# qitianwu/SGFormer

Measured on NVIDIA H100. Metric: nodes/sec fwd+bwd, higher is better.
Workload: dtype bf16

## Files before the change

sgformer_b200/csrc/common.cuh:

```cuda
#pragma once
#include <cuda.h>
#include <cuda_bf16.h>
#include <cuda_runtime.h>
#include <stdint.h>

#define SGF_OK 0
#define SGF_ERR_ARG (-1)
#define SGF_ERR_UNSUPPORTED (-2)
#define SGF_ERR_DRIVER (-3)

#define SGF_CUDA_TRY(expr)                        \
    do {                                          \
        cudaError_t _e = (expr);                  \
        if (_e != cudaSuccess) return (int)_e;    \
    } while (0)

#define SGF_LAUNCH_CHECK()                        \
    do {                                          \
        cudaError_t _e = cudaGetLastError();      \
        if (_e != cudaSuccess) return (int)_e;    \
    } while (0)

namespace sgf {

// ... 100 lines not shown
}
__device__ __forceinline__ void mbar_arrive(uint64_t* bar) {
    asm volatile("mbarrier.arrive.shared::cta.b64 _, [%0];" :: "r"(smem_u32(bar)) : "memory");
}
__device__ __forceinline__ bool mbar_try_wait(uint64_t* bar, uint32_t parity) {
    uint32_t ok;
    asm volatile(
        "{\n\t.reg .pred P;\n\t"
        "mbarrier.try_wait.parity.shared::cta.b64 P, [%1], %2;\n\t"
        "selp.b32 %0, 1, 0, P;\n\t}\n"
        : "=r"(ok) : "r"(smem_u32(bar)), "r"(parity) : "memory");
    return ok != 0;
}
__device__ __forceinline__ void mbar_wait(uint64_t* bar, uint32_t parity) {
    uint32_t spins = 0;
    while (!mbar_try_wait(bar, parity)) {
        if (++spins > (1u << 26)) __trap();
    }
}

__device__ __forceinline__ void tma_prefetch_desc(const void* tmap) {
    asm volatile("prefetch.tensormap [%0];" :: "l"(tmap) : "memory");
}
__device__ __forceinline__ void tma_load_2d(void* smem_dst, const void* tmap, uint64_t* bar, int32_t c0, int32_t c1) {
    asm volatile(
        "cp.async.bulk.tensor.2d.shared::cluster.global.mbarrier::complete_tx::bytes [%0], [%1, {%3, %4}], [%2];"
        :: "r"(smem_u32(smem_dst)), "l"(tmap), "r"(smem_u32(bar)), "r"(c0), "r"(c1) : "memory");
}

__device__ __forceinline__ void tma_store_2d(const void* tmap, const void* smem_src, int32_t c0, int32_t c1) {
    asm volatile("cp.async.bulk.tensor.2d.global.shared::cta.bulk_group [%0, {%2, %3}], [%1];"
                 :: "l"(tmap), "r"(smem_u32(smem_src)), "r"(c0), "r"(c1) : "memory");
}
__device__ __forceinline__ void cp_async16(void* smem_dst, const void* gsrc) {
    const uint32_t s = static_cast<uint32_t>(__cvta_generic_to_shared(smem_dst));
    asm volatile("cp.async.cg.shared.global [%0], [%1], 16;" ::"r"(s), "l"(gsrc) : "memory");
}
__device__ __forceinline__ void cp_async_commit() { asm volatile("cp.async.commit_group;" ::: "memory"); }
template <int N>
__device__ __forceinline__ void cp_async_wait() {
    asm volatile("cp.async.wait_group %0;" ::"n"(N) : "memory");
}

__device__ __forceinline__ void bulk_commit() { asm volatile("cp.async.bulk.commit_group;" ::: "memory"); }
template <int N> __device__ __forceinline__ void bulk_wait_read() {
    asm volatile("cp.async.bulk.wait_group.read %0;" :: "n"(N) : "memory");
}
template <int N> __device__ __forceinline__ void bulk_wait() {
    asm volatile("cp.async.bulk.wait_group %0;" :: "n"(N) : "memory");
}
__device__ __forceinline__ void named_bar_sync(int id, int nthreads) {
    asm volatile("bar.sync %0, %1;" :: "r"(id), "r"(nthreads) : "memory");
}

__device__ __forceinline__ void wgmma_fence() { asm volatile("wgmma.fence.sync.aligned;" ::: "memory"); }
__device__ __forceinline__ void wgmma_commit() { asm volatile("wgmma.commit_group.sync.aligned;" ::: "memory"); }
template <int N> __device__ __forceinline__ void wgmma_wait() {
    asm volatile("wgmma.wait_group.sync.aligned %0;" :: "n"(N) : "memory");
}
template <int N> __device__ __forceinline__ void fence_regs(float (&d)[N]) {
#pragma unroll
    for (int i = 0; i < N; ++i) asm volatile("" : "+f"(d[i]) :: "memory");
}

template <int TA, int TB>
__device__ __forceinline__ void wgmma_n64(float (&d)[32], uint64_t da, uint64_t db, uint32_t scale_d) {
// ... 56 lines not shown
```

sgformer_b200/csrc/gemm_tc.cu:

```cuda
#include "common.cuh"
#include "launch_count.h"
#include "../../include/sgformer_b200.h"

#include <cstdlib>
#include <cstring>
#include <mutex>

namespace sgf {

typedef CUresult (*PFN_encodeTiled)(CUtensorMap*, CUtensorMapDataType, cuuint32_t, void*, const cuuint64_t*, const cuuint64_t*,
                                    const cuuint32_t*, const cuuint32_t*, CUtensorMapInterleave, CUtensorMapSwizzle,
                                    CUtensorMapL2promotion, CUtensorMapFloatOOBfill);
static PFN_encodeTiled get_encode() {
    static PFN_encodeTiled fn = nullptr;
    static std::once_flag once;
    std::call_once(once, [] {
        void* p = nullptr;
        cudaDriverEntryPointQueryResult q;
        if (cudaGetDriverEntryPoint("cuTensorMapEncodeTiled", &p, cudaEnableDefault, &q) == cudaSuccess &&
            q == cudaDriverEntryPointSuccess)
            fn = (PFN_encodeTiled)p;
    });
    return fn;
}
// ... 1 lines not shown
static int make_tmap_2d(CUtensorMap* tm, const void* base, int dtype, int64_t rows, int64_t cols, int64_t ld, int box_rows) {
    PFN_encodeTiled enc = get_encode();
    if (!enc) return SGF_ERR_DRIVER;
    const int es = dtype == 1 ? 2 : 4;
    if ((reinterpret_cast<uintptr_t>(base) & 15) || (ld * es) % 16 != 0 || rows <= 0 || cols <= 0 || box_rows <= 0 || box_rows > 256)
        return SGF_ERR_ARG;
    cuuint64_t gdim[2] = {(cuuint64_t)cols, (cuuint64_t)rows};
    cuuint64_t gstr[1] = {(cuuint64_t)ld * es};
    cuuint32_t box[2] = {(cuuint32_t)(128 / es), (cuuint32_t)box_rows};
    cuuint32_t estr[2] = {1u, 1u};
    CUresult r = enc(tm, dtype == 1 ? CU_TENSOR_MAP_DATA_TYPE_BFLOAT16 : CU_TENSOR_MAP_DATA_TYPE_FLOAT32, 2,
                     const_cast<void*>(base), gdim, gstr, box, estr, CU_TENSOR_MAP_INTERLEAVE_NONE,
                     CU_TENSOR_MAP_SWIZZLE_128B, CU_TENSOR_MAP_L2_PROMOTION_L2_128B, CU_TENSOR_MAP_FLOAT_OOB_FILL_NONE);
    return r == CUDA_SUCCESS ? SGF_OK : SGF_ERR_DRIVER;
}
static int make_tmap_bf16(CUtensorMap* tm, const void* base, int64_t rows, int64_t cols, int64_t ld, int box_rows) {
    return make_tmap_2d(tm, base, 1, rows, cols, ld, box_rows);
}

namespace nt {
constexpr int BM = 128, BK = 64, STAGES = 3;
constexpr int MMA_WARPS = 8;
constexpr int THREADS = 32 * (MMA_WARPS + 4);
constexpr int A_BYTES = BM * BK * 2;
constexpr int B_BYTES_MAX = (256 + 16) * BK * 2;
constexpr int STAGE_BYTES = A_BYTES + B_BYTES_MAX;
constexpr int WSTG_BYTES = 16 * 128;
constexpr int BAR_BYTES = 512;
constexpr int STAT_COLS = 1024;
constexpr int STAT_BYTES = 2 * STAT_COLS * 4;
constexpr int SMEM_BYTES = STAGES * STAGE_BYTES + MMA_WARPS * 2 * WSTG_BYTES + BAR_BYTES + STAT_BYTES + 1024;
constexpr int RES_BYTES = (256 + 16) * 256 * 2;
constexpr int RES_MAX_KB = 16;
constexpr int RES_STAGES = 3;
constexpr int SMEM_BYTES_RES = RES_BYTES + RES_STAGES * A_BYTES + MMA_WARPS * WSTG_BYTES + BAR_BYTES + STAT_BYTES + 1024;
static_assert(SMEM_BYTES <= 232448 && SMEM_BYTES_RES <= 232448, "exceeds the 227 KB of dynamic shared memory per CTA");

struct Seg {
    int a_idx, a_koff, b_idx, b_koff, k_blocks;
};
struct Params {
    int64_t rows;
    int n_out, bn_main, bn_pad, has_tail, n_blocks;
    int64_t num_tiles;
    int b_res;
    int64_t chunk;
    int n_seg, total_kb;
    Seg seg[SGF_MAX_SEG];
    int epi;
    void* out; int64_t ldo; int out_dtype;
    const float* bias;
    const void* aux; int64_t ld_aux; int aux_dtype;
    const float* row_scale;
    float alpha, beta;
    const float* alpha_dev; const float* beta_dev;
    int relu, accumulate;
    float nf; const float* nf_dev; float* den_out;
    const float* r1_row; const float* r1_col;
    int tma_store;
    float* col_sum; float* col_sumsq;
};
struct Tmaps {
    CUtensorMap a[SGF_MAX_SRC];
    CUtensorMap b[SGF_MAX_SRC];
    CUtensorMap tail;
    CUtensorMap out;
};

__device__ __forceinline__ float load1(const void* base, int dtype, int64_t off) {
    return dtype == 1 ? __bfloat162float(static_cast<const __nv_bfloat16*>(base)[off]) : static_cast<const float*>(base)[off];
}
__device__ __forceinline__ void store1(void* base, int dtype, int64_t off, float v) {
    if (dtype == 1) static_cast<__nv_bfloat16*>(base)[off] = __float2bfloat16_rn(v);
    else static_cast<float*>(base)[off] = v;
}
struct TileIter {
    const Params& p;
    bool started = false;
// ... 45 lines not shown

enum : int { F_BIAS = 1, F_AUX = 2, F_RELU = 4, F_ROWSCALE = 8, F_ACCUM = 16, F_R1 = 32, F_ATTN = 64, F_GENERIC = 128 };

template <bool GEN>
__device__ __forceinline__ void load_piece(const void* src, int dtype, int64_t ld, const int64_t* rows, const bool* row_ok,
                                           int col0, int n_out, bool nc, float* d) {
#pragma unroll
    for (int c = 0; c < 4; ++c)
#pragma unroll
        for (int s = 0; s < 2; ++s) {
            const int col = col0 + 8 * c;
            const int64_t off = rows[s] * ld + col;
            float a0 = 0.f, a1 = 0.f;
            if (!GEN) {
                if (row_ok[s]) {
                    const uint32_t* q = reinterpret_cast<const uint32_t*>(static_cast<const __nv_bfloat16*>(src) + off);
                    unpack_bf16x2(nc ? __ldg(q) : *q, a0, a1);
                }
            } else {
                if (row_ok[s] && col < n_out) a0 = load1(src, dtype, off);
                if (row_ok[s] && col + 1 < n_out) a1 = load1(src, dtype, off + 1);
            }
            d[4 * c + 2 * s] = a0;
            d[4 * c + 2 * s + 1] = a1;
        }
}

template <int F>
__global__ void __launch_bounds__(THREADS, 1) gemm_nt_kernel(const __grid_constant__ Tmaps tm, const __grid_constant__ Params p) {
    extern __shared__ uint8_t smem_raw[];
    uint8_t* smem = reinterpret_cast<uint8_t*>((reinterpret_cast<uintptr_t>(smem_raw) + 1023) & ~static_cast<uintptr_t>(1023));
    const bool res = p.b_res != 0;
    uint8_t* bres = smem;
    uint8_t* ring = res ? smem + RES_BYTES : smem;
    const int ring_stages = res ? RES_STAGES : STAGES;
    const int ring_stride = res ? A_BYTES : STAGE_BYTES;
    const int stg_per_warp = res ? 1 : 2;
    uint8_t* staging = ring + ring_stages * ring_stride;
    uint64_t* full = reinterpret_cast<uint64_t*>(staging + MMA_WARPS * stg_per_warp * WSTG_BYTES);
    uint64_t* empty = full + STAGES;
    uint64_t* bres_full = empty + STAGES;
    uint64_t* bres_empty = bres_full + RES_MAX_KB;
    float* stat_sm = reinterpret_cast<float*>(reinterpret_cast<uint8_t*>(full) + BAR_BYTES);
    static_assert((2 * STAGES + 2 * RES_MAX_KB) * 8 <= BAR_BYTES, "barrier area");
    static_assert(RES_STAGES <= STAGES, "ring barriers");
    const bool want_stats = p.col_sum != nullptr || p.col_sumsq != nullptr;

    const int warp = threadIdx.x >> 5;
    const int lane = threadIdx.x & 31;
    const uint32_t b_tx = p.bn_pad * BK * 2 + (p.has_tail ? 16 * BK * 2 : 0);
    if (want_stats)
        for (int i = threadIdx.x; i < 2 * STAT_COLS; i += THREADS) stat_sm[i] = 0.f;

    if (threadIdx.x == 0) {
        for (int i = 0; i < p.n_seg; ++i) {
            tma_prefetch_desc(&tm.a[p.seg[i].a_idx]);
            tma_prefetch_desc(&tm.b[p.seg[i].b_idx]);
        }
        if (p.has_tail) tma_prefetch_desc(&tm.tail);
        if (p.tma_store) tma_prefetch_desc(&tm.out);
        for (int s = 0; s < STAGES; ++s) { mbar_init(&full[s], 1); mbar_init(&empty[s], MMA_WARPS); }
        for (int s = 0; s < RES_MAX_KB; ++s) { mbar_init(&bres_full[s], 1); mbar_init(&bres_empty[s], MMA_WARPS); }
        fence_barrier_init();
    }
    __syncthreads();

    if (warp >= MMA_WARPS) {
        producer_regs();
        if (warp == MMA_WARPS && lane == 0) {
            int stage = 0; uint32_t phase = 0;
            TileIter ti(p);
            while (ti.next()) {
                int kbg = 0;
                for (int s = 0; s < p.n_seg; ++s) {
                    const Seg sg = p.seg[s];
                    for (int kb = 0; kb < sg.k_blocks; ++kb, ++kbg) {
                        mbar_wait(&empty[stage], phase ^ 1);
                        uint8_t* sa = ring + stage * ring_stride;
                        if (!res) {
                            uint8_t* sb = sa + A_BYTES;
                            mbar_arrive_expect_tx(&full[stage], A_BYTES + b_tx);
                            tma_load_2d(sa, &tm.a[sg.a_idx], &full[stage], sg.a_koff + kb * BK, ti.m_blk * BM);
                            tma_load_2d(sb, &tm.b[sg.b_idx], &full[stage], sg.b_koff + kb * BK, ti.n_blk * p.bn_main);
                            if (p.has_tail) tma_load_2d(sb + p.bn_pad * BK * 2, &tm.tail, &full[stage], sg.b_koff + kb * BK, 0);
                        } else {
                            mbar_arrive_expect_tx(&full[stage], A_BYTES);
                            tma_load_2d(sa, &tm.a[sg.a_idx], &full[stage], sg.a_koff + kb * BK, ti.m_blk * BM);
                            if (ti.first) {
                                mbar_wait(&bres_empty[kbg], (uint32_t)(ti.group & 1) ^ 1);
                                uint8_t* sb = bres + (size_t)kbg * b_tx;
                                mbar_arrive_expect_tx(&bres_full[kbg], b_tx);
                                tma_load_2d(sb, &tm.b[sg.b_idx], &bres_full[kbg], sg.b_koff + kb * BK, ti.n_blk * p.bn_main);
                                if (p.has_tail) tma_load_2d(sb + p.bn_pad * BK * 2, &tm.tail, &bres_full[kbg], sg.b_koff + kb * BK, 0);
                            }
// ... 9 lines not shown

    constexpr bool GEN = (F & F_GENERIC) != 0;
    const bool f_bias = GEN ? p.bias != nullptr : (F & F_BIAS) != 0;
    const bool f_aux = GEN ? p.aux != nullptr : (F & F_AUX) != 0;
    const bool f_relu = GEN ? p.relu != 0 : (F & F_RELU) != 0;
    const bool f_rs = GEN ? p.row_scale != nullptr : (F & F_ROWSCALE) != 0;
    const bool f_acc = GEN ? p.accumulate != 0 : (F & F_ACCUM) != 0;
    const bool f_r1 = GEN ? p.r1_row != nullptr : (F & F_R1) != 0;
    const bool f_attn = GEN ? (p.epi == SGF_EPI_ATTN_APPLY || p.epi == SGF_EPI_ATTN_GRAM) : (F & F_ATTN) != 0;
    const bool f_tma = GEN ? p.tma_store != 0 : true;
    const bool f_stats = GEN ? want_stats : false;
    const int out_dtype = GEN ? p.out_dtype : 1;
    const int wg = warp >> 2;
    const int wq = warp & 3;
    const int rr = lane >> 2;
    const int cq = 2 * (lane & 3);
    float alpha = p.alpha, beta = p.beta;
    if (p.alpha_dev) alpha *= *p.alpha_dev;
    if (p.beta_dev) beta *= *p.beta_dev;
    const float nfv = (f_attn && p.nf_dev) ? *p.nf_dev : p.nf;
    const int GW = out_dtype == 1 ? 64 : 32;
    const int ppg = GW / 32;
    const int n_pieces = (p.bn_main + 31) / 32;
    const int nch = p.bn_pad / 64;
    uint8_t* wstg = staging + warp * stg_per_warp * WSTG_BYTES;
    const uint32_t a_off = wg * 64 * BK * 2;

    float acc[4][32];
    float acct[8];
    uint32_t gcount = 0;
    int stage = 0; uint32_t phase = 0;
    TileIter ti(p);
    while (ti.next()) {
        for (int kbg = 0; kbg < p.total_kb; ++kbg) {
            if (res && ti.first) mbar_wait(&bres_full[kbg], (uint32_t)(ti.group & 1));
            mbar_wait(&full[stage], phase);
            const uint32_t sa = smem_u32(ring + stage * ring_stride) + a_off;
            const uint32_t sb = res ? smem_u32(bres) + (uint32_t)kbg * b_tx : smem_u32(ring + stage * ring_stride) + A_BYTES;
            wgmma_fence();
#pragma unroll
            for (int k = 0; k < BK / 16; ++k) {
                const uint64_t da = make_smem_desc_sw128(sa + k * 32, 16, 1024);
                const uint32_t sc = (kbg > 0 || k > 0) ? 1u : 0u;
#pragma unroll
                for (int j = 0; j < 4; ++j)
                    if (j < nch) wgmma_n64<0, 0>(acc[j], da, make_smem_desc_sw128(sb + j * 8192 + k * 32, 16, 1024), sc);
                if (p.has_tail) wgmma_n16<0, 0>(acct, da, make_smem_desc_sw128(sb + p.bn_pad * BK * 2 + k * 32, 16, 1024), sc);
            }
            wgmma_commit();
            wgmma_wait<0>();
#pragma unroll
            for (int j = 0; j < 4; ++j) fence_regs(acc[j]);
            fence_regs(acct);
            __syncwarp();
            if (lane == 0) {
                mbar_arrive(&empty[stage]);
                if (res && ti.last) mbar_arrive(&bres_empty[kbg]);
            }
            if (++stage == ring_stages) { stage = 0; phase ^= 1; }
        }

        const int m_blk = ti.m_blk, n_blk = ti.n_blk;
        const int64_t row_w = (int64_t)m_blk * BM + wg * 64 + wq * 16;
        const int64_t rows[2] = {row_w + rr, row_w + rr + 8};
        const bool row_ok[2] = {rows[0] < p.rows, rows[1] < p.rows};
        const int col_base = n_blk * p.bn_main;
        float rs[2] = {1.f, 1.f}, r1r[2] = {0.f, 0.f}, inv_den[2] = {1.f, 1.f};
#pragma unroll
        for (int s = 0; s < 2; ++s) {
            if (f_rs && row_ok[s]) rs[s] = p.row_scale[rows[s]];
            if (f_r1 && row_ok[s]) r1r[s] = p.r1_row[rows[s]];
        }
        if (f_attn) {
#pragma unroll
            for (int s = 0; s < 2; ++s) {
                const float den = __shfl_sync(0xffffffffu, acct[2 * s], lane & ~3) + nfv;
                inv_den[s] = 1.f / den;
                if (row_ok[s] && p.den_out && n_blk == 0 && (lane & 3) == 0) p.den_out[rows[s]] = den;
            }
        }
#pragma unroll
        for (int pc = 0; pc < 8; ++pc) {
            if (pc >= n_pieces) break;
            const int g = pc / ppg, pp = pc % ppg;
            const uint32_t buf = stg_per_warp == 2 ? (gcount & 1) : 0;
            if (f_tma && pp == 0) {
                if (lane == 0) {
                    if (stg_per_warp == 2) bulk_wait_read<1>(); else bulk_wait_read<0>();
                }
                __syncwarp();
            }
            float v[16];
#pragma unroll
            for (int i = 0; i < 16; ++i) v[i] = acc[pc >> 1][(pc & 1) * 16 + i];
            const int col0 = col_base + pc * 32 + cq;
            float ax[16], old[16];
            if (f_aux) load_piece<GEN>(p.aux, p.aux_dtype, p.ld_aux, rows, row_ok, col0, p.n_out, true, ax);
            if (f_acc) load_piece<GEN>(p.out, out_dtype, p.ldo, rows, row_ok, col0, p.n_out, false, old);
#pragma unroll
// ... 56 lines not shown
                        float s1 = 0.f, s2 = 0.f;
                        for (int r = 0; r < 16 && r < valid_rows; ++r) {
                            float x;
                            if (out_dtype == 1) {
                                const int chunk = (cg >> 3) ^ (r & 7);
                                x = __bfloat162float(*reinterpret_cast<const __nv_bfloat16*>(tile + r * 128 + chunk * 16 + (cg & 7) * 2));
                            } else {
                                const int chunk = (cg >> 2) ^ (r & 7);
                                x = *reinterpret_cast<const float*>(tile + r * 128 + chunk * 16 + (cg & 3) * 4);
                            }
                            s1 += x;
                            s2 += x * x;
                        }
                        atomicAdd(&stat_sm[colg], s1);
                        atomicAdd(&stat_sm[STAT_COLS + colg], s2);
                    }
                }
                ++gcount;
            }
        }
    }
    if (f_tma && lane == 0) bulk_wait<0>();
    if (f_stats) {
        named_bar_sync(3, 32 * MMA_WARPS);
        for (int i = threadIdx.x; i < p.n_out; i += 32 * MMA_WARPS) {
            if (p.col_sum) atomicAdd(&p.col_sum[i], stat_sm[i]);
            if (p.col_sumsq) atomicAdd(&p.col_sumsq[i], stat_sm[STAT_COLS + i]);
        }
    }
}
}

constexpr int FLUSH_KB = 16;
template <int BATCH>
__device__ __forceinline__ void flush_acc(float (&acc)[4][32], float* ws, int mp, int mrow, int cq, int j0, int ncols, bool add) {
#pragma unroll
    for (int j = 0; j < 4; ++j) {
        if (j < j0) continue;
#pragma unroll
        for (int i0 = 0; i0 < 32; i0 += BATCH) {
            float old[BATCH];
#pragma unroll
            for (int q = 0; q < BATCH; ++q) {
                const int i = i0 + q, col = 64 * j + 8 * (i >> 2) + cq + (i & 1);
                old[q] = (add && col < ncols) ? ws[(int64_t)col * mp + mrow + 8 * ((i >> 1) & 1)] : 0.f;
            }
#pragma unroll
            for (int q = 0; q < BATCH; ++q) {
                const int i = i0 + q, col = 64 * j + 8 * (i >> 2) + cq + (i & 1);
                if (col < ncols) ws[(int64_t)col * mp + mrow + 8 * ((i >> 1) & 1)] = add ? old[q] + acc[j][i] : acc[j][i];
                acc[j][i] = 0.f;
            }
        }
    }
}

namespace tn {
constexpr int BKN = 64, STAGES = 4, MMA_WARPS = 8, THREADS = 32 * (MMA_WARPS + 4);
constexpr int CHUNK_BYTES = 64 * BKN * 2;
constexpr int A_BYTES = 2 * CHUNK_BYTES;
constexpr int B_BYTES = 4 * CHUNK_BYTES;
constexpr int STAGE_BYTES = A_BYTES + B_BYTES;
constexpr int BAR_BYTES = 256;
constexpr int SMEM_BYTES = STAGES * STAGE_BYTES + BAR_BYTES + 1024;

struct Params {
    int64_t rows;
    int m, n, mp, n_chunks, un;
    int64_t kb_total;
    float* ws;
    int n_pairs;
    int a_off[SGF_TN_MAX_PAIRS], b_off[SGF_TN_MAX_PAIRS];
};
struct Tmaps {
    CUtensorMap a, b;
};

__global__ void __launch_bounds__(THREADS, 1) gemm_tn_kernel(const __grid_constant__ Tmaps tm, const __grid_constant__ Params p) {
    extern __shared__ uint8_t smem_raw[];
    uint8_t* smem = reinterpret_cast<uint8_t*>((reinterpret_cast<uintptr_t>(smem_raw) + 1023) & ~static_cast<uintptr_t>(1023));
    uint64_t* full = reinterpret_cast<uint64_t*>(smem + STAGES * STAGE_BYTES);
    uint64_t* empty = full + STAGES;

    const int warp = threadIdx.x >> 5;
    const int lane = threadIdx.x & 31;
    const int64_t per = p.kb_total / gridDim.y, rem = p.kb_total % gridDim.y;
    const int64_t kb0 = blockIdx.y * per + (blockIdx.y < rem ? blockIdx.y : rem);
    const int64_t kb1 = kb0 + per + (blockIdx.y < rem ? 1 : 0);
    const int m0 = blockIdx.x * 128;
    const int a_chunks = (p.m - m0) >= 128 ? 2 : ((p.m - m0) + 63) / 64;

    if (threadIdx.x == 0) {
        tma_prefetch_desc(&tm.a);
        tma_prefetch_desc(&tm.b);
        for (int s = 0; s < STAGES; ++s) { mbar_init(&full[s], 1); mbar_init(&empty[s], MMA_WARPS); }
        fence_barrier_init();
    }
    __syncthreads();

    if (warp >= MMA_WARPS) {
        producer_regs();
        if (warp == MMA_WARPS && lane == 0) {
            const uint32_t stage_tx = (a_chunks + p.n_chunks) * CHUNK_BYTES;
            int stage = 0; uint32_t phase = 0;
            for (int64_t kb = kb0; kb < kb1; ++kb) {
                for (int pr = 0; pr < p.n_pairs; ++pr) {
                    mbar_wait(&empty[stage], phase ^ 1);
                    uint8_t* sa = smem + stage * STAGE_BYTES;
                    uint8_t* sb = sa + A_BYTES;
                    mbar_arrive_expect_tx(&full[stage], stage_tx);
                    for (int c = 0; c < a_chunks; ++c)
                        tma_load_2d(sa + c * CHUNK_BYTES, &tm.a, &full[stage], p.a_off[pr] + m0 + c * 64, (int32_t)(kb * BKN));
                    for (int c = 0; c < p.n_chunks; ++c)
                        tma_load_2d(sb + c * CHUNK_BYTES, &tm.b, &full[stage], p.b_off[pr] + c * 64, (int32_t)(kb * BKN));
                    if (++stage == STAGES) { stage = 0; phase ^= 1; }
                }
            }
        }
        return;
    }
    consumer_regs();

    const int wg = warp >> 2, wq = warp & 3;
    const bool active = wg < a_chunks;
    float acc[4][32];
#pragma unroll
    for (int j = 0; j < 4; ++j)
#pragma unroll
        for (int i = 0; i < 32; ++i) acc[j][i] = 0.f;
    float* ws = p.ws + (int64_t)blockIdx.y * p.un * p.mp;
    const int mrow = m0 + wg * 64 + wq * 16 + (lane >> 2);
    const int cq = 2 * (lane & 3);
    bool flushed = false;
    int stage = 0; uint32_t phase = 0;
    for (int64_t kb = kb0; kb < kb1; ++kb) {
        for (int pr = 0; pr < p.n_pairs; ++pr) {
            mbar_wait(&full[stage], phase);
            if (active) {
                const uint32_t sa = smem_u32(smem + stage * STAGE_BYTES) + wg * CHUNK_BYTES;
                const uint32_t sb = smem_u32(smem + stage * STAGE_BYTES) + A_BYTES;
                wgmma_fence();
#pragma unroll
                for (int k = 0; k < BKN / 16; ++k) {
                    const uint64_t da = make_smem_desc_sw128(sa + k * 2048, CHUNK_BYTES, 1024);
#pragma unroll
                    for (int j = 0; j < 4; ++j)
                        if (j < p.n_chunks) wgmma_n64<1, 1>(acc[j], da, make_smem_desc_sw128(sb + j * CHUNK_BYTES + k * 2048, CHUNK_BYTES, 1024), 1u);
                }
                wgmma_commit();
                wgmma_wait<0>();
#pragma unroll
                for (int j = 0; j < 4; ++j) fence_regs(acc[j]);
            }
            __syncwarp();
            if (lane == 0) mbar_arrive(&empty[stage]);
            if (++stage == STAGES) { stage = 0; phase ^= 1; }
        }
        if (active && (kb - kb0 + 1) % FLUSH_KB == 0 && kb + 1 < kb1) {
            flush_acc<16>(acc, ws, p.mp, mrow, cq, 0, p.un, flushed);
            flushed = true;
        }
    }
    flush_acc<16>(acc, ws, p.mp, mrow, cq, 0, p.un, flushed);
}

__global__ void tn_reduce_kernel(const float* __restrict__ ws, int nparts, int mp, int un, int m, int n, float alpha,
                                 const float* __restrict__ alpha_dev, float beta, float* __restrict__ out, int64_t ldo, int transpose_out) {
    const int64_t total = (int64_t)n * mp;
    const float a = alpha * (alpha_dev ? *alpha_dev : 1.f);
    for (int64_t t = (int64_t)blockIdx.x * blockDim.x + threadIdx.x; t < total; t += (int64_t)gridDim.x * blockDim.x) {
        const int j = (int)(t / mp), i = (int)(t % mp);
        if (i >= m) continue;
        float s = 0.f;
        for (int c = 0; c < nparts; ++c) s += ws[((int64_t)c * un + j) * mp + i];
        float* o = transpose_out ? &out[(int64_t)j * ldo + i] : &out[(int64_t)i * ldo + j];
        *o = a * s + (beta != 0.f ? beta * *o : 0.f);
    }
}
}
namespace gramk {
constexpr int BKN = 64, MMA_WARPS = 8, THREADS = 32 * (MMA_WARPS + 4);
constexpr int CHUNK_BYTES = 64 * BKN * 2;
constexpr int ONES_BYTES = CHUNK_BYTES;
constexpr int BAR_BYTES = 256;
constexpr int SMEM_BUDGET = 200 * 1024;
constexpr int MAX_STAGES = 8;

struct Params {
    int64_t rows, kb_total;
    int h, chunks, m_blocks, un, mp, n_planes, stages;
    int plane_off[3];
    int n_pairs, pa[6], pb[6];
    float* ws;
};

__global__ void __launch_bounds__(THREADS, 1) gram_kernel(const __grid_constant__ CUtensorMap tm, const __grid_constant__ Params p) {
    extern __shared__ uint8_t smem_raw[];
    uint8_t* smem = reinterpret_cast<uint8_t*>((reinterpret_cast<uintptr_t>(smem_raw) + 1023) & ~static_cast<uintptr_t>(1023));
    const int c0 = blockIdx.x;
    const int nld = p.chunks - c0;
    const int plane_bytes = nld * CHUNK_BYTES;
    const int stage_stride = p.n_planes * p.chunks * CHUNK_BYTES;
    uint8_t* ones = smem + p.stages * stage_stride;
    uint64_t* full = reinterpret_cast<uint64_t*>(ones + ONES_BYTES);
    uint64_t* empty = full + MAX_STAGES;
    static_assert(2 * MAX_STAGES * 8 <= BAR_BYTES, "barrier area");

    const int warp = threadIdx.x >> 5;
    const int lane = threadIdx.x & 31;
    const int64_t per = p.kb_total / gridDim.y, rem = p.kb_total % gridDim.y;
    const int64_t kb0 = blockIdx.y * per + (blockIdx.y < rem ? blockIdx.y : rem);
    const int64_t kb1 = kb0 + per + (blockIdx.y < rem ? 1 : 0);

    for (int i = threadIdx.x; i < ONES_BYTES / 4; i += THREADS) reinterpret_cast<uint32_t*>(ones)[i] = 0x3F803F80u;
    if (threadIdx.x == 0) {
        tma_prefetch_desc(&tm);
        for (int s = 0; s < p.stages; ++s) { mbar_init(&full[s], 1); mbar_init(&empty[s], MMA_WARPS); }
        fence_barrier_init();
    }
    fence_proxy_async_smem();
    __syncthreads();

    if (warp >= MMA_WARPS) {
        producer_regs();
        if (warp == MMA_WARPS && lane == 0) {
            int stage = 0; uint32_t phase = 0;
            for (int64_t kb = kb0; kb < kb1; ++kb) {
                mbar_wait(&empty[stage], phase ^ 1);
                uint8_t* sa = smem + stage * stage_stride;
                mbar_arrive_expect_tx(&full[stage], (uint32_t)(p.n_planes * plane_bytes));
                for (int pl = 0; pl < p.n_planes; ++pl)
                    for (int c = 0; c < nld; ++c)
                        tma_load_2d(sa + pl * plane_bytes + c * CHUNK_BYTES, &tm, &full[stage], p.plane_off[pl] + (c0 + c) * 64, (int32_t)(kb * BKN));
                if (++stage == p.stages) { stage = 0; phase ^= 1; }
            }
        }
        return;
    }
    consumer_regs();

    const int wg = warp >> 2, wq = warp & 3;
    const int ic = wg == 0 ? blockIdx.x : 2 * p.m_blocks - 1 - blockIdx.x;
    const bool active = ic < p.chunks;
    float acc[4][32], accs[8];
#pragma unroll
    for (int j = 0; j < 4; ++j)
#pragma unroll
        for (int i = 0; i < 32; ++i) acc[j][i] = 0.f;
#pragma unroll
    for (int i = 0; i < 8; ++i) accs[i] = 0.f;
    const uint32_t s_ones = smem_u32(ones);
    float* ws = p.ws + (int64_t)blockIdx.y * (p.un + 1) * p.mp;
    const int mrow = ic * 64 + wq * 16 + (lane >> 2);
    const int cq = 2 * (lane & 3);
    bool flushed = false;
    auto flush = [&]() {
        flush_acc<8>(acc, ws, p.mp, mrow, cq, ic, p.un, flushed);
        if (cq == 0) {
            float* w = ws + (int64_t)p.un * p.mp + mrow;
            w[0] = flushed ? w[0] + accs[0] : accs[0];
            w[8] = flushed ? w[8] + accs[2] : accs[2];
        }
#pragma unroll
        for (int i = 0; i < 8; ++i) accs[i] = 0.f;
        flushed = true;
    };
    int stage = 0; uint32_t phase = 0;
    for (int64_t kb = kb0; kb < kb1; ++kb) {
        mbar_wait(&full[stage], phase);
        if (active) {
            const uint32_t sa = smem_u32(smem + stage * stage_stride);
            wgmma_fence();
            for (int pr = 0; pr < p.n_pairs; ++pr) {
                const uint32_t a0 = sa + p.pa[pr] * plane_bytes + (ic - c0) * CHUNK_BYTES, b0 = sa + p.pb[pr] * plane_bytes;
#pragma unroll
                for (int k = 0; k < BKN / 16; ++k) {
                    const uint64_t da = make_smem_desc_sw128(a0 + k * 2048, CHUNK_BYTES, 1024);
#pragma unroll
                    for (int j = 0; j < 4; ++j)
                        if (j >= ic && j < p.chunks)
                            wgmma_n64<1, 1>(acc[j], da, make_smem_desc_sw128(b0 + (j - c0) * CHUNK_BYTES + k * 2048, CHUNK_BYTES, 1024), 1u);
                }
            }
            for (int pl = 0; pl < p.n_planes; ++pl) {
                const uint32_t a0 = sa + pl * plane_bytes + (ic - c0) * CHUNK_BYTES;
#pragma unroll
                for (int k = 0; k < BKN / 16; ++k)
                    wgmma_n16<1, 1>(accs, make_smem_desc_sw128(a0 + k * 2048, CHUNK_BYTES, 1024),
                                    make_smem_desc_sw128(s_ones + k * 2048, CHUNK_BYTES, 1024), 1u);
            }
            wgmma_commit();
            wgmma_wait<0>();
#pragma unroll
            for (int j = 0; j < 4; ++j) fence_regs(acc[j]);
            fence_regs(accs);
        }
        __syncwarp();
        if (lane == 0) mbar_arrive(&empty[stage]);
        if (++stage == p.stages) { stage = 0; phase ^= 1; }
        if (active && (kb - kb0 + 1) % FLUSH_KB == 0 && kb + 1 < kb1) flush();
    }
    if (active) flush();
}

__global__ void gram_reduce_kernel(const float* __restrict__ ws, int nparts, int un, int mp, int h, float* __restrict__ G,
                                   int64_t ldg, float* __restrict__ s) {
    const int total = h * h + h;
    for (int t = blockIdx.x * blockDim.x + threadIdx.x; t < total; t += gridDim.x * blockDim.x) {
        int i, c;
        if (t < h * h) {
            const int r = t / h, q = t % h;
            const bool upper = (q >> 6) >= (r >> 6);
            i = upper ? r : q;
            c = upper ? q : r;
        } else {
            i = t - h * h;
            c = un;
        }
        float acc = 0.f;
        for (int part = 0; part < nparts; ++part) acc += ws[((int64_t)part * (un + 1) + c) * mp + i];
        if (t < h * h) G[(int64_t)(t / h) * ldg + t % h] = acc;
        else s[i] = acc;
    }
}
}
}

using namespace sgf;

extern "C" int sgf_gemm_nt(const sgf_gemm_nt_args* a, void* stream) {
    if (!a || a->rows < 0 || a->n_out <= 0 || a->n_seg <= 0 || a->n_seg > SGF_MAX_SEG || a->n_a <= 0 || a->n_a > SGF_MAX_SRC ||
        a->n_b <= 0 || a->n_b > SGF_MAX_SRC || !a->out)
        return SGF_ERR_ARG;
// ... 50 lines not shown
        }
        p.num_tiles = m_blocks * p.n_blocks;
    }
    int rc;
    for (int i = 0; i < a->n_a; ++i)
        if ((rc = make_tmap_bf16(&tm.a[i], a->a[i], a->rows, a->a_cols[i], a->lda[i], nt::BM))) return rc;
    for (int i = 0; i < a->n_b; ++i)
        if ((rc = make_tmap_bf16(&tm.b[i], a->b[i], a->n_out, a->b_cols[i], a->ldb[i], p.bn_pad))) return rc;
    if (has_tail && (rc = make_tmap_bf16(&tm.tail, a->b_tail, 16, a->b_cols[0], a->ldb_tail, 16))) return rc;

    p.epi = a->epi;
    p.out = a->out; p.ldo = a->ldo; p.out_dtype = a->out_dtype;
    p.bias = a->bias;
    p.aux = a->aux; p.ld_aux = a->ld_aux; p.aux_dtype = a->aux_dtype;
    p.row_scale = a->row_scale;
    p.alpha = a->alpha; p.beta = a->beta; p.alpha_dev = a->alpha_dev; p.beta_dev = a->beta_dev;
    p.relu = a->relu; p.accumulate = a->accumulate;
    p.nf = a->nf; p.nf_dev = a->nf_dev; p.den_out = a->den_out;
    p.r1_row = a->r1_row; p.r1_col = a->r1_col;
    {
        const int es = a->out_dtype == 1 ? 2 : 4;
        p.tma_store = ((reinterpret_cast<uintptr_t>(a->out) & 15) == 0 && (a->ldo * es) % 16 == 0) ? 1 : 0;
        if (p.tma_store && (rc = make_tmap_2d(&tm.out, a->out, a->out_dtype, a->rows, a->n_out, a->ldo, 16))) return rc;
        p.col_sum = a->col_sum; p.col_sumsq = a->col_sumsq;
        if ((p.col_sum || p.col_sumsq) && (!p.tma_store || a->n_out > nt::STAT_COLS)) return SGF_ERR_UNSUPPORTED;
    }

    {
        const int64_t b_tx = (int64_t)(p.bn_pad + (has_tail ? 16 : 0)) * nt::BK * 2;
        const bool fits = p.total_kb <= nt::RES_MAX_KB && b_tx * p.total_kb <= nt::RES_BYTES;
        if (a->schedule == SGF_GEMM_RESIDENT_B && !fits) return SGF_ERR_UNSUPPORTED;
        p.b_res = (fits && (a->schedule == SGF_GEMM_RESIDENT_B || (a->schedule == SGF_GEMM_AUTO && p.n_blocks == 1))) ? 1 : 0;
        p.chunk = p.n_blocks == 1 ? (int64_t)1 << 40 : 4;
    }
    const int64_t work = p.b_res ? m_blocks : p.num_tiles;
    const int64_t grid = work < num_sms() ? work : num_sms();
    const int smem_bytes = p.b_res ? nt::SMEM_BYTES_RES : nt::SMEM_BYTES;

    int feat = (a->bias ? nt::F_BIAS : 0) | (a->aux ? nt::F_AUX : 0) | (a->relu ? nt::F_RELU : 0) |
               (a->row_scale ? nt::F_ROWSCALE : 0) | (a->accumulate ? nt::F_ACCUM : 0) | (a->r1_row ? nt::F_R1 : 0) |
               (a->epi != SGF_EPI_AFFINE ? nt::F_ATTN : 0);
    const bool al16 = (!a->bias || (reinterpret_cast<uintptr_t>(a->bias) & 15) == 0) &&
                      (!a->r1_col || (reinterpret_cast<uintptr_t>(a->r1_col) & 15) == 0) &&
                      (!a->aux || (a->aux_dtype == 1 && (reinterpret_cast<uintptr_t>(a->aux) & 15) == 0 && (a->ld_aux * 2) % 16 == 0));
    const bool fast_ok = p.tma_store && a->out_dtype == 1 && a->n_out % 32 == 0 && al16 && !p.col_sum && !p.col_sumsq &&
                         p.n_blocks * p.bn_main == a->n_out;
    static const bool no_special = [] { const char* e = getenv("SGF_GEMM_NT_GENERIC"); return e && e[0] == '1'; }();
    if (!fast_ok || no_special) feat = nt::F_GENERIC;
    const int smem_max = nt::SMEM_BYTES > nt::SMEM_BYTES_RES ? nt::SMEM_BYTES : nt::SMEM_BYTES_RES;
#define SGF_NT_CASE(FEAT)                                                                                                   \
    case (FEAT): {                                                                                                         \
        static bool attr_set = false;                                                                                      \
        if (!attr_set) {                                                                                                   \
            SGF_CUDA_TRY(cudaFuncSetAttribute(nt::gemm_nt_kernel<(FEAT)>, cudaFuncAttributeMaxDynamicSharedMemorySize,     \
                                              smem_max));                                                                  \
            attr_set = true;                                                                                               \
        }                                                                                                                  \
        nt::gemm_nt_kernel<(FEAT)><<<(unsigned)grid, nt::THREADS, smem_bytes, (cudaStream_t)stream>>>(tm, p);              \
        launched = true;                                                                                                   \
    } break;
    for (int attempt = 0; attempt < 2; ++attempt) {
        bool launched = false;
        switch (feat) {
            SGF_NT_CASE(0)
            SGF_NT_CASE(nt::F_BIAS)
            SGF_NT_CASE(nt::F_BIAS | nt::F_RELU)
            SGF_NT_CASE(nt::F_ROWSCALE)
            SGF_NT_CASE(nt::F_ACCUM)
            SGF_NT_CASE(nt::F_AUX)
            SGF_NT_CASE(nt::F_AUX | nt::F_ACCUM)
            SGF_NT_CASE(nt::F_AUX | nt::F_BIAS)
            SGF_NT_CASE(nt::F_AUX | nt::F_R1)
            SGF_NT_CASE(nt::F_AUX | nt::F_ATTN)
            SGF_NT_CASE(nt::F_BIAS | nt::F_ATTN)
            SGF_NT_CASE(nt::F_BIAS | nt::F_R1)
            SGF_NT_CASE(nt::F_BIAS | nt::F_R1 | nt::F_ACCUM)
            SGF_NT_CASE(nt::F_GENERIC)
            default: break;
        }
        if (launched) break;
        feat = nt::F_GENERIC;
    }
// ... 20 lines not shown
    cudaStream_t st = (cudaStream_t)stream;
    tn::Params p;
    memset(&p, 0, sizeof(p));
    p.rows = a->rows; p.m = a->m; p.n = a->n;
    const int m_blocks = (a->m + 127) / 128;
    p.mp = m_blocks * 128;
    p.un = (a->n + 15) / 16 * 16;
    p.n_chunks = (p.un + 63) / 64;
    p.kb_total = (a->rows + tn::BKN - 1) / tn::BKN;
    p.ws = (float*)a->ws;
    if (a->n_pairs < 0 || a->n_pairs > SGF_TN_MAX_PAIRS) return SGF_ERR_ARG;
    p.n_pairs = a->n_pairs > 0 ? a->n_pairs : 1;
    int64_t a_span = a->m, b_span = a->n;
    for (int i = 0; i < p.n_pairs; ++i) {
        p.a_off[i] = a->n_pairs > 0 ? a->a_off[i] : 0;
        p.b_off[i] = a->n_pairs > 0 ? a->b_off[i] : 0;
        if (p.a_off[i] < 0 || p.b_off[i] < 0 || p.a_off[i] % 64 || p.b_off[i] % 64) return SGF_ERR_ARG;
        if (p.a_off[i] + a->m > a_span) a_span = p.a_off[i] + a->m;
        if (p.b_off[i] + a->n > b_span) b_span = p.b_off[i] + a->n;
    }
    const int mp = p.mp;
    int grid = 0;
    if (a->rows > 0) {
        size_t need = 0;
        sgf_gemm_tn_ws_bytes(a->m, a->n, a->rows, &need);
        if (a->ws_bytes < need) return SGF_ERR_ARG;
        tn::Tmaps tm;
        memset(&tm, 0, sizeof(tm));
        int rc;
        if ((rc = make_tmap_bf16(&tm.a, a->a, a->rows, a_span, a->lda, tn::BKN))) return rc;
        if ((rc = make_tmap_bf16(&tm.b, a->b, a->rows, b_span, a->ldb, tn::BKN))) return rc;
        static bool attr_set = false;
        if (!attr_set) {
            SGF_CUDA_TRY(cudaFuncSetAttribute(tn::gemm_tn_kernel, cudaFuncAttributeMaxDynamicSharedMemorySize, tn::SMEM_BYTES));
            attr_set = true;
        }
        grid = tn_splits(p.kb_total, m_blocks);
        tn::gemm_tn_kernel<<<dim3(m_blocks, grid), tn::THREADS, tn::SMEM_BYTES, st>>>(tm, p);
        SGF_LAUNCH_CHECK(); count_launch();
    }
    int64_t total = (int64_t)a->n * mp;
    int rgrid = (int)((total + 255) / 256);
    tn::tn_reduce_kernel<<<rgrid, 256, 0, st>>>(p.ws, grid, mp, p.un, a->m, a->n, a->alpha, a->alpha_dev, a->beta, a->out, a->ldo,
                                                a->transpose_out);
    SGF_LAUNCH_CHECK(); count_launch();
    return SGF_OK;
}


static int gram_geometry(int h, int planes, int64_t rows, gramk::Params& p) {
    if (h <= 0 || h > 256 || (planes != 1 && planes != 3) || rows < 0) return SGF_ERR_ARG;
    memset(&p, 0, sizeof(p));
    p.rows = rows; p.h = h;
    p.chunks = (h + 63) / 64;
    p.m_blocks = h > 128 ? 2 : 1;
    p.un = (h + 15) / 16 * 16;
    p.mp = p.m_blocks * 128;
    p.n_planes = planes;
    p.kb_total = (rows + gramk::BKN - 1) / gramk::BKN;
    p.stages = gramk::SMEM_BUDGET / (planes * p.chunks * gramk::CHUNK_BYTES);
    if (p.stages > gramk::MAX_STAGES) p.stages = gramk::MAX_STAGES;
    if (p.stages < 2) return SGF_ERR_UNSUPPORTED;
    return SGF_OK;
}

extern "C" int sgf_gram_ws_bytes(int32_t h, int32_t planes, int64_t rows, size_t* bytes) {
    gramk::Params p;
    int rc = gram_geometry(h, planes, rows, p);
    if (rc || !bytes) return rc ? rc : SGF_ERR_ARG;
    *bytes = (size_t)tn_splits(p.kb_total, p.m_blocks) * (p.un + 1) * p.mp * sizeof(float);
    return SGF_OK;
// ... 43 lines not shown
```

Measured before the change: 11.25 million.

## Deepen GEMM pipelines, overlap wgmma in resident mode, and move partial flushes on-chip

The NT GEMM's resident-B path now sizes its A ring from the leftover shared memory, up to 8 stages, and keeps one wgmma group in flight, releasing the previous stage instead of waiting for each group to drain. Accumulate and aux rows are prefetched into L2 at tile start. The TN GEMM sizes its stage count dynamically and keeps periodic partial sums in shared memory instead of read-modify-write passes over the global workspace. The gram kernel's flushes use red.global.add. These changes add more shared memory use and complexity, plus diagnostic compile flags for disabling loads or MMAs.

```diff
diff --git a/sgformer_b200/csrc/common.cuh b/sgformer_b200/csrc/common.cuh
--- a/sgformer_b200/csrc/common.cuh
+++ b/sgformer_b200/csrc/common.cuh
@@ -156,6 +156,9 @@
     asm volatile("cp.async.bulk.tensor.2d.global.shared::cta.bulk_group [%0, {%2, %3}], [%1];"
                  :: "l"(tmap), "r"(smem_u32(smem_src)), "r"(c0), "r"(c1) : "memory");
 }
+__device__ __forceinline__ void bulk_prefetch_l2(const void* gsrc, uint32_t bytes) {
+    asm volatile("cp.async.bulk.prefetch.L2.global [%0], %1;" :: "l"(gsrc), "r"(bytes) : "memory");
+}
 __device__ __forceinline__ void cp_async16(void* smem_dst, const void* gsrc) {
     const uint32_t s = static_cast<uint32_t>(__cvta_generic_to_shared(smem_dst));
     asm volatile("cp.async.cg.shared.global [%0], [%1], 16;" ::"r"(s), "l"(gsrc) : "memory");
diff --git a/sgformer_b200/csrc/gemm_tc.cu b/sgformer_b200/csrc/gemm_tc.cu
--- a/sgformer_b200/csrc/gemm_tc.cu
+++ b/sgformer_b200/csrc/gemm_tc.cu
@@ -57,9 +57,11 @@
 constexpr int SMEM_BYTES = STAGES * STAGE_BYTES + MMA_WARPS * 2 * WSTG_BYTES + BAR_BYTES + STAT_BYTES + 1024;
 constexpr int RES_BYTES = (256 + 16) * 256 * 2;
 constexpr int RES_MAX_KB = 16;
-constexpr int RES_STAGES = 3;
-constexpr int SMEM_BYTES_RES = RES_BYTES + RES_STAGES * A_BYTES + MMA_WARPS * WSTG_BYTES + BAR_BYTES + STAT_BYTES + 1024;
-static_assert(SMEM_BYTES <= 232448 && SMEM_BYTES_RES <= 232448, "exceeds the 227 KB of dynamic shared memory per CTA");
+constexpr int RES_MIN_STAGES = 3, RING_MAX = 8;
+constexpr int SMEM_LIMIT = 232448;
+constexpr int RES_FIXED_BYTES = MMA_WARPS * WSTG_BYTES + BAR_BYTES + STAT_BYTES + 1024;
+constexpr int SMEM_BYTES_RES = RES_BYTES + RES_MIN_STAGES * A_BYTES + RES_FIXED_BYTES;
+static_assert(SMEM_BYTES <= SMEM_LIMIT && SMEM_BYTES_RES <= SMEM_LIMIT, "exceeds the 227 KB of dynamic shared memory per CTA");
 
 struct Seg {
     int a_idx, a_koff, b_idx, b_koff, k_blocks;
@@ -69,6 +71,7 @@
     int n_out, bn_main, bn_pad, has_tail, n_blocks;
     int64_t num_tiles;
     int b_res;
+    int res_bytes, ring_stages;
     int64_t chunk;
     int n_seg, total_kb;
     Seg seg[SGF_MAX_SEG];
@@ -180,18 +183,18 @@
     uint8_t* smem = reinterpret_cast<uint8_t*>((reinterpret_cast<uintptr_t>(smem_raw) + 1023) & ~static_cast<uintptr_t>(1023));
     const bool res = p.b_res != 0;
     uint8_t* bres = smem;
-    uint8_t* ring = res ? smem + RES_BYTES : smem;
-    const int ring_stages = res ? RES_STAGES : STAGES;
+    uint8_t* ring = res ? smem + p.res_bytes : smem;
+    const int ring_stages = res ? p.ring_stages : STAGES;
     const int ring_stride = res ? A_BYTES : STAGE_BYTES;
     const int stg_per_warp = res ? 1 : 2;
     uint8_t* staging = ring + ring_stages * ring_stride;
     uint64_t* full = reinterpret_cast<uint64_t*>(staging + MMA_WARPS * stg_per_warp * WSTG_BYTES);
-    uint64_t* empty = full + STAGES;
-    uint64_t* bres_full = empty + STAGES;
+    uint64_t* empty = full + RING_MAX;
+    uint64_t* bres_full = empty + RING_MAX;
     uint64_t* bres_empty = bres_full + RES_MAX_KB;
     float* stat_sm = reinterpret_cast<float*>(reinterpret_cast<uint8_t*>(full) + BAR_BYTES);
-    static_assert((2 * STAGES + 2 * RES_MAX_KB) * 8 <= BAR_BYTES, "barrier area");
-    static_assert(RES_STAGES <= STAGES, "ring barriers");
+    static_assert((2 * RING_MAX + 2 * RES_MAX_KB) * 8 <= BAR_BYTES, "barrier area");
+    static_assert(STAGES <= RING_MAX, "ring barriers");
     const bool want_stats = p.col_sum != nullptr || p.col_sumsq != nullptr;
 
     const int warp = threadIdx.x >> 5;
@@ -207,7 +210,7 @@
         }
         if (p.has_tail) tma_prefetch_desc(&tm.tail);
         if (p.tma_store) tma_prefetch_desc(&tm.out);
-        for (int s = 0; s < STAGES; ++s) { mbar_init(&full[s], 1); mbar_init(&empty[s], MMA_WARPS); }
+        for (int s = 0; s < ring_stages; ++s) { mbar_init(&full[s], 1); mbar_init(&empty[s], MMA_WARPS); }
         for (int s = 0; s < RES_MAX_KB; ++s) { mbar_init(&bres_full[s], 1); mbar_init(&bres_empty[s], MMA_WARPS); }
         fence_barrier_init();
     }
@@ -283,6 +286,14 @@
     int stage = 0; uint32_t phase = 0;
     TileIter ti(p);
     while (ti.next()) {
+        const int m_blk = ti.m_blk, n_blk = ti.n_blk;
+        const int64_t row_w = (int64_t)m_blk * BM + wg * 64 + wq * 16;
+        const int col_base = n_blk * p.bn_main;
+        if (!GEN && (f_acc || f_aux) && lane < 16 && row_w + lane < p.rows) {
+            if (f_acc) bulk_prefetch_l2(static_cast<const __nv_bfloat16*>(p.out) + (row_w + lane) * p.ldo + col_base, p.bn_main * 2);
+            if (f_aux) bulk_prefetch_l2(static_cast<const __nv_bfloat16*>(p.aux) + (row_w + lane) * p.ld_aux + col_base, p.bn_main * 2);
+        }
+        int prev = 0;
         for (int kbg = 0; kbg < p.total_kb; ++kbg) {
             if (res && ti.first) mbar_wait(&bres_full[kbg], (uint32_t)(ti.group & 1));
             mbar_wait(&full[stage], phase);
@@ -299,23 +310,28 @@
                 if (p.has_tail) wgmma_n16<0, 0>(acct, da, make_smem_desc_sw128(sb + p.bn_pad * BK * 2 + k * 32, 16, 1024), sc);
             }
             wgmma_commit();
-            wgmma_wait<0>();
-#pragma unroll
-            for (int j = 0; j < 4; ++j) fence_regs(acc[j]);
-            fence_regs(acct);
+            if (res) wgmma_wait<1>();
+            else wgmma_wait<0>();
             __syncwarp();
-            if (lane == 0) {
-                mbar_arrive(&empty[stage]);
-                if (res && ti.last) mbar_arrive(&bres_empty[kbg]);
-            }
+            if (lane == 0 && (kbg > 0 || !res)) {
+                mbar_arrive(&empty[res ? prev : stage]);
+                if (res && ti.last) mbar_arrive(&bres_empty[kbg - 1]);
+            }
+            prev = stage;
             if (++stage == ring_stages) { stage = 0; phase ^= 1; }
         }
-
-        const int m_blk = ti.m_blk, n_blk = ti.n_blk;
-        const int64_t row_w = (int64_t)m_blk * BM + wg * 64 + wq * 16;
+        wgmma_wait<0>();
+#pragma unroll
+        for (int j = 0; j < 4; ++j) fence_regs(acc[j]);
+        fence_regs(acct);
+        __syncwarp();
+        if (lane == 0 && res) {
+            mbar_arrive(&empty[prev]);
+            if (ti.last) mbar_arrive(&bres_empty[p.total_kb - 1]);
+        }
+
         const int64_t rows[2] = {row_w + rr, row_w + rr + 8};
         const bool row_ok[2] = {rows[0] < p.rows, rows[1] < p.rows};
-        const int col_base = n_blk * p.bn_main;
         float rs[2] = {1.f, 1.f}, r1r[2] = {0.f, 0.f}, inv_den[2] = {1.f, 1.f};
 #pragma unroll
         for (int s = 0; s < 2; ++s) {
@@ -438,37 +454,37 @@
 }
 
 constexpr int FLUSH_KB = 16;
-template <int BATCH>
-__device__ __forceinline__ void flush_acc(float (&acc)[4][32], float* ws, int mp, int mrow, int cq, int j0, int ncols, bool add) {
+#ifndef SGF_TN_DIAG
+#define SGF_TN_DIAG 0
+#endif
+
+__device__ __forceinline__ void red_add_f32(float* p, float v) {
+    asm volatile("red.global.add.f32 [%0], %1;" :: "l"(p), "f"(v) : "memory");
+}
+__device__ __forceinline__ void flush_acc_red(float (&acc)[4][32], float* ws, int mp, int mrow, int cq, int j0, int ncols, bool add) {
 #pragma unroll
     for (int j = 0; j < 4; ++j) {
         if (j < j0) continue;
 #pragma unroll
-        for (int i0 = 0; i0 < 32; i0 += BATCH) {
-            float old[BATCH];
-#pragma unroll
-            for (int q = 0; q < BATCH; ++q) {
-                const int i = i0 + q, col = 64 * j + 8 * (i >> 2) + cq + (i & 1);
-                old[q] = (add && col < ncols) ? ws[(int64_t)col * mp + mrow + 8 * ((i >> 1) & 1)] : 0.f;
-            }
-#pragma unroll
-            for (int q = 0; q < BATCH; ++q) {
-                const int i = i0 + q, col = 64 * j + 8 * (i >> 2) + cq + (i & 1);
-                if (col < ncols) ws[(int64_t)col * mp + mrow + 8 * ((i >> 1) & 1)] = add ? old[q] + acc[j][i] : acc[j][i];
-                acc[j][i] = 0.f;
-            }
+        for (int i = 0; i < 32; ++i) {
+            const int col = 64 * j + 8 * (i >> 2) + cq + (i & 1);
+            float* w = ws + (int64_t)col * mp + mrow + 8 * ((i >> 1) & 1);
+            if (col < ncols) {
+                if (add) red_add_f32(w, acc[j][i]);
+                else *w = acc[j][i];
+            }
+            acc[j][i] = 0.f;
         }
     }
 }
 
 namespace tn {
-constexpr int BKN = 64, STAGES = 4, MMA_WARPS = 8, THREADS = 32 * (MMA_WARPS + 4);
+constexpr int BKN = 64, MAX_STAGES = 8, MMA_WARPS = 8, THREADS = 32 * (MMA_WARPS + 4);
 constexpr int CHUNK_BYTES = 64 * BKN * 2;
 constexpr int A_BYTES = 2 * CHUNK_BYTES;
-constexpr int B_BYTES = 4 * CHUNK_BYTES;
-constexpr int STAGE_BYTES = A_BYTES + B_BYTES;
+constexpr int PART_CHUNK_BYTES = 32 * 32 * MMA_WARPS * 4;
 constexpr int BAR_BYTES = 256;
-constexpr int SMEM_BYTES = STAGES * STAGE_BYTES + BAR_BYTES + 1024;
+constexpr int SMEM_LIMIT = 232448;
 
 struct Params {
     int64_t rows;
@@ -476,6 +492,7 @@
     int64_t kb_total;
     float* ws;
     int n_pairs;
+    int stages, stage_bytes;
     int a_off[SGF_TN_MAX_PAIRS], b_off[SGF_TN_MAX_PAIRS];
 };
 struct Tmaps {
@@ -485,8 +502,10 @@
 __global__ void __launch_bounds__(THREADS, 1) gemm_tn_kernel(const __grid_constant__ Tmaps tm, const __grid_constant__ Params p) {
     extern __shared__ uint8_t smem_raw[];
     uint8_t* smem = reinterpret_cast<uint8_t*>((reinterpret_cast<uintptr_t>(smem_raw) + 1023) & ~static_cast<uintptr_t>(1023));
-    uint64_t* full = reinterpret_cast<uint64_t*>(smem + STAGES * STAGE_BYTES);
-    uint64_t* empty = full + STAGES;
+    uint8_t* part_base = smem + p.stages * p.stage_bytes;
+    uint64_t* full = reinterpret_cast<uint64_t*>(part_base + p.n_chunks * PART_CHUNK_BYTES);
+    uint64_t* empty = full + MAX_STAGES;
+    static_assert(2 * MAX_STAGES * 8 <= BAR_BYTES, "barrier area");
 
     const int warp = threadIdx.x >> 5;
     const int lane = threadIdx.x & 31;
@@ -499,7 +518,7 @@
     if (threadIdx.x == 0) {
         tma_prefetch_desc(&tm.a);
         tma_prefetch_desc(&tm.b);
-        for (int s = 0; s < STAGES; ++s) { mbar_init(&full[s], 1); mbar_init(&empty[s], MMA_WARPS); }
+        for (int s = 0; s < p.stages; ++s) { mbar_init(&full[s], 1); mbar_init(&empty[s], MMA_WARPS); }
         fence_barrier_init();
     }
     __syncthreads();
@@ -512,14 +531,19 @@
             for (int64_t kb = kb0; kb < kb1; ++kb) {
                 for (int pr = 0; pr < p.n_pairs; ++pr) {
                     mbar_wait(&empty[stage], phase ^ 1);
-                    uint8_t* sa = smem + stage * STAGE_BYTES;
+                    uint8_t* sa = smem + stage * p.stage_bytes;
                     uint8_t* sb = sa + A_BYTES;
+#if SGF_TN_DIAG == 3
+                    mbar_arrive(&full[stage]);
+                    (void)sb; (void)stage_tx;
+#else
                     mbar_arrive_expect_tx(&full[stage], stage_tx);
                     for (int c = 0; c < a_chunks; ++c)
                         tma_load_2d(sa + c * CHUNK_BYTES, &tm.a, &full[stage], p.a_off[pr] + m0 + c * 64, (int32_t)(kb * BKN));
                     for (int c = 0; c < p.n_chunks; ++c)
                         tma_load_2d(sb + c * CHUNK_BYTES, &tm.b, &full[stage], p.b_off[pr] + c * 64, (int32_t)(kb * BKN));
-                    if (++stage == STAGES) { stage = 0; phase ^= 1; }
+#endif
+                    if (++stage == p.stages) { stage = 0; phase ^= 1; }
                 }
             }
         }
@@ -537,14 +561,15 @@
     float* ws = p.ws + (int64_t)blockIdx.y * p.un * p.mp;
     const int mrow = m0 + wg * 64 + wq * 16 + (lane >> 2);
     const int cq = 2 * (lane & 3);
+    float* part = reinterpret_cast<float*>(part_base) + threadIdx.x;
     bool flushed = false;
     int stage = 0; uint32_t phase = 0;
     for (int64_t kb = kb0; kb < kb1; ++kb) {
         for (int pr = 0; pr < p.n_pairs; ++pr) {
             mbar_wait(&full[stage], phase);
-            if (active) {
-                const uint32_t sa = smem_u32(smem + stage * STAGE_BYTES) + wg * CHUNK_BYTES;
-                const uint32_t sb = smem_u32(smem + stage * STAGE_BYTES) + A_BYTES;
+            if (active && SGF_TN_DIAG != 2) {
+                const uint32_t sa = smem_u32(smem + stage * p.stage_bytes) + wg * CHUNK_BYTES;
+                const uint32_t sb = smem_u32(smem + stage * p.stage_bytes) + A_BYTES;
                 wgmma_fence();
 #pragma unroll
                 for (int k = 0; k < BKN / 16; ++k) {
@@ -560,14 +585,32 @@
             }
             __syncwarp();
             if (lane == 0) mbar_arrive(&empty[stage]);
-            if (++stage == STAGES) { stage = 0; phase ^= 1; }
-        }
-        if (active && (kb - kb0 + 1) % FLUSH_KB == 0 && kb + 1 < kb1) {
-            flush_acc<16>(acc, ws, p.mp, mrow, cq, 0, p.un, flushed);
+            if (++stage == p.stages) { stage = 0; phase ^= 1; }
+        }
+        if (active && (kb - kb0 + 1) % FLUSH_KB == 0 && kb + 1 < kb1 && SGF_TN_DIAG != 1) {
+#pragma unroll
+            for (int j = 0; j < 4; ++j) {
+                if (j >= p.n_chunks) continue;
+#pragma unroll
+                for (int i = 0; i < 32; ++i) {
+                    float& q = part[(32 * j + i) * (32 * MMA_WARPS)];
+                    q = flushed ? q + acc[j][i] : acc[j][i];
+                    acc[j][i] = 0.f;
+                }
+            }
             flushed = true;
         }
     }
-    flush_acc<16>(acc, ws, p.mp, mrow, cq, 0, p.un, flushed);
+#pragma unroll
+    for (int j = 0; j < 4; ++j)
+#pragma unroll
+        for (int i = 0; i < 32; ++i) {
+            const int col = 64 * j + 8 * (i >> 2) + cq + (i & 1);
+            if (col < p.un) {
+                const float v = acc[j][i];
+                ws[(int64_t)col * p.mp + mrow + 8 * ((i >> 1) & 1)] = flushed ? part[(32 * j + i) * (32 * MMA_WARPS)] + v : v;
+            }
+        }
 }
 
 __global__ void tn_reduce_kernel(const float* __restrict__ ws, int nparts, int mp, int un, int m, int n, float alpha,
@@ -634,10 +677,15 @@
             for (int64_t kb = kb0; kb < kb1; ++kb) {
                 mbar_wait(&empty[stage], phase ^ 1);
                 uint8_t* sa = smem + stage * stage_stride;
+#if SGF_TN_DIAG == 3
+                mbar_arrive(&full[stage]);
+                (void)sa;
+#else
                 mbar_arrive_expect_tx(&full[stage], (uint32_t)(p.n_planes * plane_bytes));
                 for (int pl = 0; pl < p.n_planes; ++pl)
                     for (int c = 0; c < nld; ++c)
                         tma_load_2d(sa + pl * plane_bytes + c * CHUNK_BYTES, &tm, &full[stage], p.plane_off[pl] + (c0 + c) * 64, (int32_t)(kb * BKN));
+#endif
                 if (++stage == p.stages) { stage = 0; phase ^= 1; }
             }
         }
@@ -661,11 +709,11 @@
     const int cq = 2 * (lane & 3);
     bool flushed = false;
     auto flush = [&]() {
-        flush_acc<8>(acc, ws, p.mp, mrow, cq, ic, p.un, flushed);
+        flush_acc_red(acc, ws, p.mp, mrow, cq, ic, p.un, flushed);
         if (cq == 0) {
             float* w = ws + (int64_t)p.un * p.mp + mrow;
-            w[0] = flushed ? w[0] + accs[0] : accs[0];
-            w[8] = flushed ? w[8] + accs[2] : accs[2];
+            if (flushed) { red_add_f32(w, accs[0]); red_add_f32(w + 8, accs[2]); }
+            else { w[0] = accs[0]; w[8] = accs[2]; }
         }
 #pragma unroll
         for (int i = 0; i < 8; ++i) accs[i] = 0.f;
@@ -674,7 +722,7 @@
     int stage = 0; uint32_t phase = 0;
     for (int64_t kb = kb0; kb < kb1; ++kb) {
         mbar_wait(&full[stage], phase);
-        if (active) {
+        if (active && SGF_TN_DIAG != 2) {
             const uint32_t sa = smem_u32(smem + stage * stage_stride);
             wgmma_fence();
             for (int pr = 0; pr < p.n_pairs; ++pr) {
@@ -704,7 +752,7 @@
         __syncwarp();
         if (lane == 0) mbar_arrive(&empty[stage]);
         if (++stage == p.stages) { stage = 0; phase ^= 1; }
-        if (active && (kb - kb0 + 1) % FLUSH_KB == 0 && kb + 1 < kb1) flush();
+        if (active && (kb - kb0 + 1) % FLUSH_KB == 0 && kb + 1 < kb1 && SGF_TN_DIAG != 1) flush();
     }
     if (active) flush();
 }
@@ -821,10 +869,14 @@
         if (a->schedule == SGF_GEMM_RESIDENT_B && !fits) return SGF_ERR_UNSUPPORTED;
         p.b_res = (fits && (a->schedule == SGF_GEMM_RESIDENT_B || (a->schedule == SGF_GEMM_AUTO && p.n_blocks == 1))) ? 1 : 0;
         p.chunk = p.n_blocks == 1 ? (int64_t)1 << 40 : 4;
+        p.res_bytes = (int)(b_tx * p.total_kb);
+        const int st = (nt::SMEM_LIMIT - p.res_bytes - nt::RES_FIXED_BYTES) / nt::A_BYTES;
+        p.ring_stages = st < nt::RING_MAX ? st : nt::RING_MAX;
+        if (p.b_res && p.ring_stages < nt::RES_MIN_STAGES) return SGF_ERR_UNSUPPORTED;
     }
     const int64_t work = p.b_res ? m_blocks : p.num_tiles;
     const int64_t grid = work < num_sms() ? work : num_sms();
-    const int smem_bytes = p.b_res ? nt::SMEM_BYTES_RES : nt::SMEM_BYTES;
+    const int smem_bytes = p.b_res ? p.res_bytes + p.ring_stages * nt::A_BYTES + nt::RES_FIXED_BYTES : nt::SMEM_BYTES;
 
     int feat = (a->bias ? nt::F_BIAS : 0) | (a->aux ? nt::F_AUX : 0) | (a->relu ? nt::F_RELU : 0) |
                (a->row_scale ? nt::F_ROWSCALE : 0) | (a->accumulate ? nt::F_ACCUM : 0) | (a->r1_row ? nt::F_R1 : 0) |
@@ -836,7 +888,7 @@
                          p.n_blocks * p.bn_main == a->n_out;
     static const bool no_special = [] { const char* e = getenv("SGF_GEMM_NT_GENERIC"); return e && e[0] == '1'; }();
     if (!fast_ok || no_special) feat = nt::F_GENERIC;
-    const int smem_max = nt::SMEM_BYTES > nt::SMEM_BYTES_RES ? nt::SMEM_BYTES : nt::SMEM_BYTES_RES;
+    const int smem_max = nt::SMEM_LIMIT;
 #define SGF_NT_CASE(FEAT)                                                                                                   \
     case (FEAT): {                                                                                                         \
         static bool attr_set = false;                                                                                      \
@@ -923,11 +975,16 @@
         if ((rc = make_tmap_bf16(&tm.b, a->b, a->rows, b_span, a->ldb, tn::BKN))) return rc;
         static bool attr_set = false;
         if (!attr_set) {
-            SGF_CUDA_TRY(cudaFuncSetAttribute(tn::gemm_tn_kernel, cudaFuncAttributeMaxDynamicSharedMemorySize, tn::SMEM_BYTES));
+            SGF_CUDA_TRY(cudaFuncSetAttribute(tn::gemm_tn_kernel, cudaFuncAttributeMaxDynamicSharedMemorySize, tn::SMEM_LIMIT));
             attr_set = true;
         }
+        p.stage_bytes = tn::A_BYTES + p.n_chunks * tn::CHUNK_BYTES;
+        const int fixed = p.n_chunks * tn::PART_CHUNK_BYTES + tn::BAR_BYTES + 1024;
+        const int stages = (tn::SMEM_LIMIT - fixed) / p.stage_bytes;
+        p.stages = stages < tn::MAX_STAGES ? stages : tn::MAX_STAGES;
+        if (p.stages < 2) return SGF_ERR_UNSUPPORTED;
         grid = tn_splits(p.kb_total, m_blocks);
-        tn::gemm_tn_kernel<<<dim3(m_blocks, grid), tn::THREADS, tn::SMEM_BYTES, st>>>(tm, p);
+        tn::gemm_tn_kernel<<<dim3(m_blocks, grid), tn::THREADS, p.stages * p.stage_bytes + fixed, st>>>(tm, p);
         SGF_LAUNCH_CHECK(); count_launch();
     }
     int64_t total = (int64_t)a->n * mp;
```

Result: faster. 11.60 million, median of 6 (+3.1%).
